# brianz98/A-Fortran-Electronic-Structure-Program

Hardware: AMD Instinct MI355X
Metric: CCSD iter wall-time (s) + (T) wall-time (s); fp64 TFLOP/s vs MFMA peak (higher is better)
Workload: dtype f64; 1 GPU; cfg5: nocc=20 nvirt=200, synthetic hashed ERIs scale 0.005; step = 1 CCSD iteration (replicated) + full (T) over i<=j<=k sharded across ranks; nocc=20, nvirt=200, triples=1540, parallelism=(T) ijk-shard x1, CCSD replicas

## Files before the change

### a-fortran-electronic-structure-program_amd/csrc/ccsd.h

```cpp
#pragma once
#include "afesp_internal.h"

namespace afesp {

struct DiisRing {
    int nerr = 0, nact = 0, it = 0;
    int64_t nvec = 0;
    double *amp = nullptr;
    double *amp_s = nullptr;
    double *hist_t = nullptr, *hist_e = nullptr;
    double *coef = nullptr;
    double *bmat = nullptr;
    bool tail_pending = false;
    int tail_slot = 0, tail_n = 0;
    double tail_b[256];
};
void diis_alloc(Context& cx, DiisRing& r, int diis_nerr);
void diis_save(Context& cx, DiisRing& r);
void diis_update(Context& cx, DiisRing& r);

struct CCState : DiisRing {
    int o = 0, v = 0;
    bool ready = false;
    double* e = nullptr;
    Tensor v_oovv, v_ovov, v_vvov, v_oovo, v_oooo, v_vvvv, w_oovv, w_vvov, w_oovo;
    Tensor D1, D2, t1, t2, t2_old, r1, r2;
    double* pp = nullptr;
    double* r2_sh = nullptr;
    double* r1_sh = nullptr;
    bool sharded = false;
    int sh_rank = 0, sh_world = 1;
    int64_t* pp_tab = nullptr;
    bool pp_sym = false;
    double *pp_vs = nullptr, *pp_va = nullptr, *pp_cs = nullptr, *pp_ca = nullptr, *pp_ps = nullptr, *pp_pa = nullptr;
    int64_t pp_ks = 0, pp_ka = 0, pp_ns = 0, pp_na = 0, pp_kn = 0;
    int64_t pp_lds = 0, pp_lda = 0;
    double *pp_ts = nullptr, *pp_ta = nullptr;
    double *oo_vs = nullptr, *oo_va = nullptr;
    double *oo_xs = nullptr, *oo_xa = nullptr;
    bool cs_packed = false;
    double* r1x = nullptr;
    bool r1x_valid = false;
    int hist_plain = 0;
    bool amps_touched = true;
    int64_t pp_nm = 0;
    double *ov_ws = nullptr, *ov_wa = nullptr;
    Tensor I_vo, I_vv, I_oo_p, I_oo, c, asym, x_voov, I_oooo, I_ovov, I_voov, I_ooov_p;
    Tensor z_ooov;
    double energy = 0.0, energy_old = 0.0, rms = 0.0;
    void* tplan = nullptr;
    Tensor I_vovv_pp, I_ooov_pp;
    const double* eri_src = nullptr;
    double* eri_own = nullptr;
    bool have_cr = false;
    int64_t amp_epoch = 0, cr_epoch = 0;
    void* ring = nullptr;
    bool partials_live = false;
    int64_t frozen_id = 0;
};
void triples_plan_free(CCState& s);

bool ring_tg_applies(const CCState& s);
bool ring_tg_pack(Context& cx, CCState& s);
void ring_tg_intermediates(Context& cx, CCState& s);
void ring_tg_residual(Context& cx, CCState& s);
void ring_tg_materialize(Context& cx, CCState& s, const Tensor& I_ovov_out, const Tensor& I_voov_out);
bool ring_live(const CCState& s);
bool ring_res_live(const CCState& s);
void ring_res_clear(CCState& s);
void ring_invalidate(CCState& s);
void ring_reinit(CCState& s);
const double* ring_Y(const CCState& s);
void ring_free(Context& cx, CCState& s);

void ccsd_init(Context& cx, CCState& s, int o, int v, const double* eri_mo_dev, const double* e_host, int diis_nerr);
bool ccsd_can_reinit(const CCState& s, int o, int v, int diis_nerr);
void ccsd_need_vvvv(Context& cx, CCState& s);
void ccsd_refresh_sharding(Context& cx, CCState& s);
bool ccsd_uses_lanes(const CCState& s);
void ccsd_diis_save(Context& cx, CCState& s);
void ccsd_intermediates(Context& cx, CCState& s, bool save_for_diis = false);
void ccsd_amplitudes(Context& cx, CCState& s, bool defer_update = false);
void ccsd_tail_launch(Context& cx, CCState& s);
int ccsd_tail_read(Context& cx, CCState& s, double e_tol, double t_tol);
void ccsd_pp_ladder(Context& cx, CCState& s);
void ccsd_ooov_pair_form(Context& cx, CCState& s, double* out = nullptr, int64_t a0 = 0, int64_t a1 = 0);
const double* ccsd_residual_full(Context& cx, CCState& s, bool r2);
void ccsd_build_I_vovv_p(Context& cx, CCState& s, const Tensor& out);
// ... 16 lines not shown
```

### a-fortran-electronic-structure-program_amd/csrc/ccsd.hip

```cpp
#include <algorithm>
#include <cmath>
#include <cstdlib>
#include <cstring>

#include "ccsd.h"
#include "comm.h"
#include "fused.h"

namespace afesp {

static inline int64_t tri64(int64_t i, int64_t j) { return i >= j ? i * (i + 1) / 2 + j : j * (j + 1) / 2 + i; }

bool ccsd_can_reinit(const CCState& s, int o, int v, int diis_nerr)
{
    if (!knobs().cc_reinit) return false;
    return s.ready && s.o == o && s.v == v && s.nerr == diis_nerr && s.pp_sym == pp_sym_pays(o, v);
}

void ccsd_init(Context& cx, CCState& s, int o, int v, const double* eri_mo_dev, const double* e_host, int diis_nerr)
{
    if (o <= 0 || v <= 0) throw Error(1, "ccsd_init: need at least one occupied and one virtual orbital");
    const bool again = ccsd_can_reinit(s, o, v, diis_nerr);
    if (again) {
        cx.quiesce();
// ... 32 lines not shown
    const int64_t fid = ++cx.amp_clock;
    for (Tensor* t : {&s.v_oovv, &s.v_ovov, &s.v_vvov, &s.v_oovo, &s.v_oooo, &s.w_oovv, &s.w_oovo}) t->frozen = fid;
    s.frozen_id = fid;
    if (again && s.w_vvov.d) {
        k_antisym_pair(cx, s.w_vvov.d, s.v_vvov.d, s.v, s.v, s.o, s.v, 0);
        s.w_vvov.frozen = fid;
    }
    T(s.D1, {O, V}); T(s.D2, {O, O, V, V});
    k_denominators(cx, s.D1.d, s.D2.d, s.e, o, v);
    s.nvec = ov + o2v2;
    if (!again) {
        s.amp = cx.alloc(s.nvec);
        s.t1 = view(s.amp, {O, V}); s.t2 = view(s.amp + ov, {O, O, V, V});
        double* res = cx.alloc(s.nvec);
        s.r1 = view(res, {O, V}); s.r2 = view(res + ov, {O, O, V, V});
    } else {
        AFESP_HIP(hipMemsetAsync(s.t1.d, 0, sizeof(double) * ov, cx.stream));
        AFESP_HIP(hipMemsetAsync(s.t2_old.d, 0, sizeof(double) * o2v2, cx.stream));
    }
    T(s.t2_old, {O, O, V, V});
    T(s.I_vo, {V, O}); T(s.I_vv, {V, V}); T(s.I_oo_p, {O, O}); T(s.I_oo, {O, O});
    T(s.c, {O, O, V, V}); T(s.asym, {O, O, V, V}); T(s.x_voov, {V, O, O, V});
    T(s.I_oooo, {O, O, O, O}); T(s.I_ovov, {O, V, O, V}); T(s.I_voov, {V, O, O, V});
    T(s.I_ooov_p, {O, O, O, V}); T(s.z_ooov, {O, O, O, V});
    {
        const int64_t np = V * (V + 1) / 2, K2 = V * V, N2 = O * O;
        A(s.pp, N2 * np + O * O * V * V + O * V);
        s.r2_sh = s.pp + N2 * np;
        s.r1_sh = s.r2_sh + O * O * V * V;
        std::vector<int64_t> tab;
        if (!s.pp_sym) {
            tab.reserve((size_t)(np + 2 * K2 + N2));
            for (int64_t b = 0; b < V; ++b)
                for (int64_t a = 0; a <= b; ++a) tab.push_back((a + V * b) * K2);
            for (int64_t k = 0; k < K2; ++k) tab.push_back(k);
            for (int64_t k = 0; k < K2; ++k) tab.push_back(N2 * k);
            for (int64_t x = 0; x < N2; ++x) tab.push_back(x);
            for (int64_t pz = 0; pz < np; ++pz) tab.push_back(N2 * pz);
        } else {
            auto even = [](int64_t x) { return (x + 1) & ~(int64_t)1; };
            const int64_t npa = V * (V - 1) / 2, ks = even(np), ka = even(npa), ns = even(O * (O + 1) / 2), na = even(O * (O - 1) / 2);
            s.pp_ks = ks; s.pp_ka = ka; s.pp_ns = ns; s.pp_na = na;
            const int64_t lds = ks + ns, lda = ka + na, kx = lds;
            s.pp_lds = lds; s.pp_lda = lda;
            const int64_t nm = std::max(np, O * V);
            s.pp_nm = nm;
            A(s.pp_vs, lds * np); A(s.pp_cs, ns * kx); A(s.pp_ps, ns * nm);
// ... 39 lines not shown
    if (s.v_vvvv.d) return;
    if (!s.eri_src)
        throw Error(1, "the <ef|ab> slice is formed on request from the packed MO integrals, and those have been replaced since "
                       "afesp_ccsd_init: initialise the solver again");
    const int64_t V = s.v;
    s.v_vvvv = cx.tensor({V, V, V, V});
    k_slice_phys(cx, s.v_vvvv.d, s.eri_src, s.v, s.v, s.v, s.v, s.o, s.o, s.o, s.o);
}

static void ccsd_need_w_vvov(Context& cx, CCState& s)
{
    if (s.w_vvov.d) return;
    s.w_vvov = cx.tensor({(int64_t)s.v, (int64_t)s.v, (int64_t)s.o, (int64_t)s.v});
    k_antisym_pair(cx, s.w_vvov.d, s.v_vvov.d, s.v, s.v, s.o, s.v, 0);
    s.w_vvov.frozen = s.frozen_id;
}

void ccsd_free(Context& cx, CCState& s)
{
    if (!s.o) return;
    if (s.eri_own) cx.release(s.eri_own);
    double* bufs[] = {s.e, s.v_oovv.d, s.v_ovov.d, s.v_vvov.d, s.v_oovo.d, s.v_oooo.d, s.v_vvvv.d, s.w_oovv.d, s.w_vvov.d,
                      s.w_oovo.d, s.D1.d, s.D2.d, s.amp, s.r1.d, s.t2_old.d, s.I_vo.d, s.I_vv.d, s.I_oo_p.d, s.I_oo.d, s.c.d,
                      s.asym.d, s.x_voov.d, s.I_oooo.d, s.I_ovov.d, s.I_voov.d, s.I_ooov_p.d, s.z_ooov.d, s.amp_s, s.hist_t,
                      s.hist_e, s.coef, s.I_vovv_pp.d, s.I_ooov_pp.d, s.pp, (double*)s.pp_tab, s.pp_vs, s.pp_va, s.pp_cs,
                      s.pp_ca, s.pp_ps, s.pp_pa, s.bmat, s.ov_ws, s.ov_wa, s.pp_ts, s.pp_ta, s.oo_vs, s.oo_va, s.oo_xs, s.oo_xa, s.r1x};
    for (double* b : bufs) cx.release(b);
    if (cx.plans.size() > 1024 || cx.plan_bytes > ((size_t)4 << 30)) cx.plan_clear();
    cx.drop_scratch();
    triples_plan_free(s);
    ring_free(cx, s);
    s = CCState();
}

void diis_alloc(Context& cx, DiisRing& s, int diis_nerr)
{
    s.nerr = diis_nerr; s.nact = 0; s.it = 0;
    if (diis_nerr >= 2) {
        if (diis_nerr > 15) throw Error(1, "ccsd_init: ccsd_diis_n_errmat > 15 is not supported");
        s.amp_s = cx.alloc(s.nvec);
        s.hist_t = cx.alloc(s.nvec * diis_nerr);
        s.hist_e = cx.alloc(s.nvec * diis_nerr);
        s.coef = cx.alloc(32);
        s.bmat = cx.alloc((int64_t)diis_nerr * diis_nerr);
    }
}

// ... 27 lines not shown
        if (knobs().cc_time_slice) { s.sharded = true; s.sh_rank = knobs().cc_time_rank; s.sh_world = knobs().cc_time_world; }
}

static void slice_bounds(const CCState& s, int64_t* v0, int64_t* v1)
{
    if (!s.sharded) { *v0 = 0; *v1 = s.v; return; }
    *v0 = (int64_t)s.v * s.sh_rank / s.sh_world;
    *v1 = (int64_t)s.v * (s.sh_rank + 1) / s.sh_world;
}

static Tensor slice_axis(Tensor t, int axis, int64_t lo, int64_t hi)
{
    t.d += lo * t.stride[axis];
    t.dim[axis] = hi - lo;
    return t;
}

void ccsd_intermediates(Context& cx, CCState& s, bool save_for_diis)
{
    auto C = [&](double al, const Tensor& A, const char* la, const Tensor& B, const char* lb, double be, const Tensor& Cc,
                 const char* lc) { contract(cx, al, A, la, B, lb, be, Cc, lc); };
    ccsd_refresh_sharding(cx, s);
    s.amps_touched = false;
    s.r1x_valid = false;
    int64_t v0, v1;
    slice_bounds(s, &v0, &v1);
    auto sl = [&](const Tensor& t, int axis) { return slice_axis(t, axis, v0, v1); };
    if (!(lanes_pay(s) || cx.rec) && ring_tg_applies(s) && ring_tg_pack(cx, s)) {}
    else k_asym_c(cx, s.asym.d, s.c.d, s.t1.d, s.t2.d, s.o, s.v);
    const bool par = lanes_pay(s) && !cx.rec;
    const bool fused = cx.rec != nullptr;
    const bool ring = !par && !fused && ring_tg_applies(s);
    if (!ring) ring_invalidate(s);
    auto lane = [&](int i) { if (par) cx.use_lane(i); };
    if (par) cx.fork(6);
    lane(0);
    C(1.0, s.w_oovv, "miea", s.t1, "me", 0.0, s.I_vo, "ai");
    lane(1);
    const bool ivv_diag = !par && !fused && s.o >= 2;
    if (!ivv_diag) {
        ccsd_need_w_vvov(cx, s);
        C(1.0, s.w_vvov, "ebma", s.t1, "me", 0.0, s.I_vv, "ba");
    }
    if (!s.sharded) C(-1.0, s.w_oovv, "mneb", s.c, "mnea", ivv_diag ? 0.0 : 1.0, s.I_vv, "ba");
    else if (v1 > v0) C(-1.0, s.w_oovv, "mneb", sl(s.c, 3), "mnea", ivv_diag ? 0.0 : 1.0, slice_axis(s.I_vv, 1, v0, v1), "ba");
    lane(0);
// ... 7 lines not shown
    }
    C(1.0, s.t1, "je", s.I_vo, "ei", 1.0, s.I_oo, "ji");
    lane(1);
    k_copy(cx, s.I_oooo.d, s.v_oooo.d, s.I_oooo.size());
    if (s.pp_sym && !par && !fused) ccsd_oooo_pair_form(cx, s);
    else C(1.0, s.c, "klef", s.v_oovv, "ijef", 1.0, s.I_oooo, "klij");
    C(1.0, s.t1, "ke", s.v_oovo, "ilej", 1.0, s.I_oooo, "klij");
    C(1.0, s.t1, "le", s.v_oovo, "jkei", 1.0, s.I_oooo, "klij");
    lane(2);
    const int64_t a_len = s.I_ovov.stride[3], a_off = v0 * a_len, a_cnt = (v1 - v0) * a_len;
    if (ivv_diag && s.sharded) {
        if (v1 > v0) C(1.0, s.t1, "je", sl(s.v_vvov, 3), "ebia", 0.0, sl(s.I_ovov, 3), "jbia");
    } else if (ivv_diag) {
        contract_pair(cx, {1.0, &s.t1, "je", &s.v_vvov, "ebia", 0.0, &s.I_ovov, "jbia"}, {1.0, &s.v_vvov, "beia", &s.t1, "je", 0.0, &s.x_voov, "bjia"});
    } else if (v1 > v0) {
        k_copy(cx, s.I_ovov.d + a_off, s.v_ovov.d + a_off, a_cnt);
        if (!ring) C(-0.5, s.v_oovv, "mibe", sl(s.c, 2), "mjae", 1.0, sl(s.I_ovov, 3), "jbia");
        C(-1.0, s.v_oovo, "mibj", sl(s.t1, 1), "ma", 1.0, sl(s.I_ovov, 3), "jbia");
        C(1.0, s.t1, "je", sl(s.v_vvov, 3), "ebia", 1.0, sl(s.I_ovov, 3), "jbia");
    }
    lane(3);
    if (s.sharded) { if (v1 > v0) C(1.0, sl(s.v_vvov, 3), "beia", s.t1, "je", 0.0, sl(s.x_voov, 3), "bjia"); }
    else if (!ivv_diag) C(1.0, s.v_vvov, "beia", s.t1, "je", 0.0, s.x_voov, "bjia");
    if (ivv_diag && v1 > v0) {
        k_ivv_diag(cx, s.I_vv.d, s.I_ovov.d, s.x_voov.d, s.o, s.v, (int)v0, (int)v1);
        k_axpby(cx, s.I_ovov.d + a_off, 1.0, s.v_ovov.d + a_off, 1.0, a_cnt);
        if (!ring) C(-0.5, s.v_oovv, "mibe", sl(s.c, 2), "mjae", 1.0, sl(s.I_ovov, 3), "jbia");
        C(-1.0, s.v_oovo, "mibj", sl(s.t1, 1), "ma", 1.0, sl(s.I_ovov, 3), "jbia");
    }
    const int x_voov_ready = par ? cx.mark() : 0;
    if (v1 > v0) {
        permute_add(cx, 1.0, sl(s.v_oovv, 2), "jiab", 0.0, sl(s.I_voov, 3), "bjia");
        if (fused) C(1.0, s.v_vvov, "beia", s.t1, "je", 1.0, s.I_voov, "bjia");
        else k_axpby(cx, s.I_voov.d + a_off, 1.0, s.x_voov.d + a_off, 1.0, a_cnt);
        if (!ring) {
            C(0.5, s.w_oovv, "imbe", sl(s.t2, 3), "mjea", 1.0, sl(s.I_voov, 3), "bjia");
            C(-0.5, s.v_oovv, "imbe", sl(s.c, 2), "mjae", 1.0, sl(s.I_voov, 3), "bjia");
        }
        C(-1.0, s.v_oovo, "imbj", sl(s.t1, 1), "ma", 1.0, sl(s.I_voov, 3), "bjia");
    }
    if (ring) ring_tg_intermediates(cx, s);
    lane(4);
    if (save_for_diis) diis_save(cx, s);
    if (fused) permute_add(cx, 1.0, s.v_oovo, "kjai", 0.0, s.z_ooov, "jkia");
    C(1.0, s.t1, "ie", s.v_oovv, "mjeb", fused ? 1.0 : 0.0, s.z_ooov, "ijmb");
    C(1.0, s.t1, "je", s.v_ovov, "mbie", 1.0, s.z_ooov, "ijmb");
    lane(5);
    permute_add(cx, 1.0, s.v_oovo, "kjai", 0.0, s.I_ooov_p, "jkia");
    if (s.sharded) {
        Tensor osh = view(cx.scratch("ooov_sh", s.I_ooov_p.size()), {(int64_t)s.o, (int64_t)s.o, (int64_t)s.o, (int64_t)s.v});
        if (v1 > v0) {
            if (s.pp_sym) {
                AFESP_HIP(hipMemsetAsync(osh.d + osh.stride[3] * v0, 0, sizeof(double) * osh.stride[3] * (v1 - v0), cx.stream));
                ccsd_ooov_pair_form(cx, s, osh.d, v0, v1);
            } else {
                C(1.0, s.t2, "jkef", sl(s.v_vvov, 3), "efia", 0.0, sl(osh, 3), "jkia");
            }
            if (par) cx.wait(x_voov_ready);
            C(1.0, s.t1, "je", sl(s.x_voov, 3), "ekia", 1.0, sl(osh, 3), "jkia");
        }
    } else if (s.pp_sym) {
        ccsd_ooov_pair_form(cx, s);
    } else {
        C(1.0, s.t2, "jkef", s.v_vvov, "efia", 1.0, s.I_ooov_p, "jkia");
// ... 179 lines not shown
    if (par) {
        r2b.d = cx.scratch(R2_LANE2, s.r2.size());
        r2c.d = cx.scratch(R2_LANE3, s.r2.size());
        r1b.d = cx.scratch(R1_LANE5, s.r1.size());
        cx.fork(6);
    }
    lane(0);
    if (!sh) C(1.0, s.t1, "ie", s.I_vv, "ea", 0.0, s.r1, "ia");
    C(-1.0, s.I_oo_p, "im", s.t1, "ma", sh ? 0.0 : 1.0, s.r1, "ia");
    C(1.0, s.asym, "miea", s.I_vo, "em", 1.0, s.r1, "ia");
    C(2.0, s.v_oovv, "miea", s.t1, "me", 1.0, s.r1, "ia");
    lane(5);
    if (par && cx.test_throw == 1) {
        cx.test_throw = 0;
        throw Error(99, "injected failure (afesp_test_inject)");
    }
    C(-1.0, s.v_ovov, "maie", s.t1, "me", par ? 0.0 : 1.0, r1b, "ia");
    C(-1.0, s.v_oovo, "mien", s.asym, "mnea", 1.0, r1b, "ia");
    if (!sh && s.r1x_valid && !par && !cx.rec) k_axpby(cx, r1b.d, 1.0, s.r1x, 1.0, r1b.size());
    else if (!sh) C(1.0, s.asym, "mief", s.v_vvov, "efma", 1.0, r1b, "ia");
    lane(1);
    const bool open_with_vvov = !par && !cx.rec && !sh;
    if (ring) ring_tg_residual(cx, s);
    if (open_with_vvov && !s.amps_touched) permute_add(cx, 1.0, s.x_voov, "bija", ring ? 1.0 : 0.0, s.r2, "ijab");
    else if (open_with_vvov) C(1.0, s.t1, "ie", s.v_vvov, "baje", ring ? 1.0 : 0.0, s.r2, "ijab");
    if (!sh) {
        C(1.0, s.t2, "ijae", s.I_vv, "eb", open_with_vvov ? 1.0 : 0.0, s.r2, "ijab");
        C(-1.0, s.t2, "miba", s.I_oo, "jm", 1.0, s.r2, "ijab");
    }
    lane(4);
    ccsd_pp_ladder(cx, s);
    lane(1);
    if (!sh && !(s.pp_sym && !cx.rec)) C(0.5, s.I_oooo, "ijmn", s.c, "mnab", 1.0, s.r2, "ijab");
    lane(2);
    if (ring) {
    } else if (!sh) {
        C(-1.0, s.t2, "mjae", s.I_ovov, "iemb", par ? 0.0 : 1.0, r2b, "ijab");
        C(-1.0, s.I_ovov, "iema", s.t2, "mjeb", 1.0, r2b, "ijab");
    } else if (v1 > v0) {
        C(-1.0, s.t2, "mjae", sl(s.I_ovov, 3), "iemb", 1.0, sl(r2s, 3), "ijab");
        C(-1.0, sl(s.I_ovov, 3), "iema", s.t2, "mjeb", 1.0, sl(r2s, 2), "ijab");
        C(1.0, s.asym, "miea", sl(s.I_voov, 3), "ejmb", 1.0, sl(r2s, 3), "ijab");
        Tensor osh = view(cx.scratch("ooov_sh", s.I_ooov_p.size()), {(int64_t)s.o, (int64_t)s.o, (int64_t)s.o, (int64_t)s.v});
        C(-1.0, s.t1, "ma", sl(osh, 3), "ijmb", 1.0, sl(r2s, 3), "ijab");
        C(1.0, s.t1, "ie", slice_axis(s.v_vvov, 0, v0, v1), "baje", 1.0, sl(r2s, 3), "ijab");
        C(1.0, s.t2, "ijae", slice_axis(s.I_vv, 1, v0, v1), "eb", 1.0, sl(r2s, 3), "ijab");
        C(-1.0, slice_axis(s.t2, 2, v0, v1), "miba", s.I_oo, "jm", 1.0, sl(r2s, 3), "ijab");
        C(0.5, s.I_oooo, "ijmn", sl(s.c, 3), "mnab", 1.0, sl(r2s, 3), "ijab");
        C(-1.0, s.t1, "ma", sl(s.z_ooov, 3), "ijmb", 1.0, sl(r2s, 3), "ijab");
        Tensor r1s = s.r1;
        r1s.d = s.r1_sh;
        C(1.0, s.t1, "ie", slice_axis(s.I_vv, 1, v0, v1), "ea", 1.0, slice_axis(r1s, 1, v0, v1), "ia");
        C(1.0, s.asym, "mief", sl(s.v_vvov, 3), "efma", 1.0, slice_axis(r1s, 1, v0, v1), "ia");
    }
    lane(3);
    if (!sh && !ring) C(1.0, s.asym, "miea", s.I_voov, "ejmb", par ? 0.0 : 1.0, r2c, "ijab");
    if (!open_with_vvov && !sh) C(1.0, s.t1, "ie", s.v_vvov, "baje", 1.0, r2c, "ijab");
    if (!sh) C(-1.0, s.t1, "ma", s.z_ooov, "ijmb", 1.0, r2c, "ijab");
    if (par) cx.join();
    if (sh) {
        const int64_t np = (int64_t)s.v * (s.v + 1) / 2;
        comm_allreduce_dev(cx, cx.comm, s.pp, (int64_t)s.o * s.o * np + s.r2.size() + s.r1.size());
        k_copy(cx, s.r2.d, s.r2_sh, s.r2.size());
        k_axpby(cx, s.r1.d, 1.0, s.r1_sh, 1.0, s.r1.size());
    }
    if (defer_update) return;
    k_t2_update(cx, s.t2.d, s.r2.d, par ? r2b.d : nullptr, par ? r2c.d : nullptr, s.v_oovv.d, s.D2.d, s.pp, s.o, s.v, s.t1.d, s.r1.d,
                par ? r1b.d : nullptr, s.D1.d, ring ? ring_Y(s) : nullptr);
}

const double* ccsd_residual_full(Context& cx, CCState& s, bool r2)
{
    const int64_t n = r2 ? s.r2.size() : s.r1.size();
    double* full = cx.scratch(r2 ? "r2_full" : "r1_full", n);
    auto add_partial = [&](const char* buf) {
        auto it = cx.cache.find(buf);
        if (s.partials_live && it != cx.cache.end()) k_axpby(cx, full, 1.0, (const double*)it->second.first, 1.0, n);
    };
    if (r2) {
        k_r2_full(cx, full, s.r2.d, s.pp, s.o, s.v);
        add_partial(R2_LANE2);
// ... 215 lines not shown
```

### a-fortran-electronic-structure-program_amd/csrc/ring.hip

```cpp
#include <algorithm>
#include <cstdlib>
#include <cstring>

#include "ccsd.h"

namespace afesp {

struct RingTg {
    int64_t ov = 0, Kc = 0, each = 0;
    double* slab = nullptr;
    double *cp, *t2p, *t2x, *asp, *nIo, *Ivo, *F1, *F2, *F3, *Y;
    uint32_t* rc32 = nullptr;
    int64_t *cm1 = nullptr, *cn1 = nullptr, *cm2 = nullptr, *cn2 = nullptr;
    int64_t* tab_block = nullptr;
    TgGroup* groups = nullptr;
    int tiles = 0, mx = 0;
    bool pairs2 = false;
    bool frozen_built = false;
    bool packed = false;
    bool live = false;
    bool res_live = false;
};

__global__ __launch_bounds__(256) void ring_tables_kernel(uint32_t* rc32, int64_t* cm1, int64_t* cn1, int64_t* cm2, int64_t* cn2, int o, int v,
                                                          int64_t Kc)
{
    const int64_t ov = (int64_t)o * v;
    for (int64_t x = (int64_t)blockIdx.x * blockDim.x + threadIdx.x; x < ov + 256; x += (int64_t)gridDim.x * blockDim.x) {
        const int64_t y = x < ov ? x : ov - 1;
        rc32[x] = (uint32_t)(8 * Kc * y);
        if (x < ov + 128) {
            const int64_t p = y % o, q = y / o;
            cm1[x] = Kc * y;
            cn1[x] = y;
// ... 51 lines not shown
        int r2 = (int)ring_div((unsigned)r, inv_np);
        const int pp = r - r2 * np;
        const int qq = (int)ring_div((unsigned)r2, a.inv_o), j = r2 - qq * o;
        const int blk = oo * (pp + P * qq);
        const double t = tile[m + o * j + blk], tt = tile[j + o * m + blk];
        const int64_t out = m + O * (p0 + pp) + a.Kc * (j + O * (q0 + qq));
        a.t2p[out] = t;
        a.asp[out] = 2.0 * t - tt;
    }
    const unsigned inv_nq = nq == 1 ? 0u : (unsigned)(((uint64_t)1 << 32) / (unsigned)nq + 1);
    for (int idx = threadIdx.x; idx < n; idx += 256) {
        int r = (int)ring_div((unsigned)idx, a.inv_o);
        const int m = idx - r * o;
        int r2 = (int)ring_div((unsigned)r, inv_nq);
        const int qq = r - r2 * nq;
        const int pp = (int)ring_div((unsigned)r2, a.inv_o), j = r2 - pp * o;
        const double t = tile[m + o * j + oo * (pp + P * qq)];
        const int64_t out = m + O * (q0 + qq) + a.Kc * (j + O * (p0 + pp));
        a.t2x[out] = t;
        a.cp[out] = t + a.t1[m + o * (p0 + pp)] * a.t1[j + o * (q0 + qq)];
    }
}

static RingTg* ring_get(Context& cx, CCState& s)
{
    if (s.ring) return (RingTg*)s.ring;
    RingTg* r = new RingTg();
    s.ring = r;
    const int64_t O = s.o, V = s.v;
    r->ov = O * V;
    r->Kc = (r->ov + TG_BK - 1) / TG_BK * TG_BK;
    r->each = r->Kc * r->ov + 2 * TG_BK;
    r->each = (r->each + 15) / 16 * 16;
    r->slab = cx.alloc(10 * r->each);
    double** bufs[10] = {&r->cp, &r->t2p, &r->t2x, &r->asp, &r->nIo, &r->Ivo, &r->F1, &r->F2, &r->F3, &r->Y};
    for (int q = 0; q < 10; ++q) *bufs[q] = r->slab + q * r->each;
    const int64_t n32 = r->ov + 256, n64 = r->ov + 128;
    int64_t* tab = cx.alloc_i64(4 * n64 + (n32 + 1) / 2 + 8);
    r->cm1 = tab; r->cn1 = tab + n64; r->cm2 = tab + 2 * n64; r->cn2 = tab + 3 * n64;
    r->rc32 = (uint32_t*)(tab + 4 * n64);
    r->tab_block = tab;
    AFESP_KLAUNCH(ring_tables_kernel, dim3((unsigned)std::min<int64_t>((n32 + 255) / 256, 4096)), dim3(256), 0, cx.stream, r->rc32, r->cm1,
                       r->cn1, r->cm2, r->cn2, s.o, s.v, r->Kc);
    AFESP_HIP(hipGetLastError());
    const int M = (int)r->ov, mt = (M + TG_BM - 1) / TG_BM, nt = (M + TG_BN - 1) / TG_BN;
    const int nk1 = (int)(r->Kc / TG_BK), gm = tgemm_group_m(M, nt);
    r->mx = nt;
    r->tiles = 2 * mt * nt;
    auto off = [&](const double* p) { return (int64_t)(p - r->slab); };
    TgGroup g[6] = {};
    auto fill = [&](TgGroup& d, const double* a1, const double* a2, const double* b1, const double* b2, const double* c, const int64_t* cn,
                    int tile0, int nk) {
        d.a1 = off(a1); d.a2 = off(a2); d.b1 = off(b1); d.b2 = off(b2); d.c0 = off(c);
        d.colB = r->rc32; d.offCn = cn;
        d.N = M; d.ntiles = nt; d.tile_start = tile0; d.nk1 = nk1; d.nk = nk;
        d.inv_width = tgemm_inverse(gm * nt);
    };
    fill(g[0], r->t2p, r->cp, r->F2, r->F3, r->Ivo, r->cn1, 0, 2 * nk1);
    fill(g[1], r->cp, r->cp, r->F1, r->F1, r->nIo, r->cn1, mt * nt, nk1);
    g[2].tile_start = 2 * mt * nt;
    fill(g[3], r->t2p, r->Ivo, r->nIo, r->asp, s.r2.d, r->cn2, 0, 2 * nk1);
    fill(g[4], r->nIo, r->nIo, r->t2x, r->t2x, r->Y, r->cn2, mt * nt, nk1);
    g[5].tile_start = 2 * mt * nt;
    r->groups = (TgGroup*)cx.alloc((int64_t)(6 * sizeof(TgGroup) / (sizeof(double)) + 1));
    AFESP_HIP(hipMemcpyAsync(r->groups, g, sizeof(g), hipMemcpyHostToDevice, cx.stream));
    AFESP_HIP(hipStreamSynchronize(cx.stream));
    r->pairs2 = (O % 2 == 0);
    return r;
}

void ring_free(Context& cx, CCState& s)
{
    RingTg* r = (RingTg*)s.ring;
    if (!r) return;
    cx.release(r->slab);
    cx.release(r->tab_block);
    cx.release(r->groups);
    delete r;
    s.ring = nullptr;
}

bool ring_live(const CCState& s) { return s.ring && ((RingTg*)s.ring)->live; }
bool ring_res_live(const CCState& s) { return s.ring && ((RingTg*)s.ring)->res_live; }
void ring_res_clear(CCState& s) { if (s.ring) ((RingTg*)s.ring)->res_live = false; }
const double* ring_Y(const CCState& s) { return ((RingTg*)s.ring)->Y; }

static Tensor kview(const RingTg* r, double* buf, const CCState& s, int pos_m, int pos_p, int pos_x, int pos_e)
{
    Tensor t;
    t.d = buf;
    t.rank = 4;
    const int64_t O = s.o, V = s.v;
    t.dim[pos_m] = O; t.stride[pos_m] = 1;
    t.dim[pos_e] = V; t.stride[pos_e] = O;
    t.dim[pos_p] = O; t.stride[pos_p] = r->Kc;
    t.dim[pos_x] = V; t.stride[pos_x] = r->Kc * O;
    return t;
}

bool ring_tg_pack(Context& cx, CCState& s)
{
    const bool off = !knobs().ring_pack;
    const int64_t oo = (int64_t)s.o * s.o;
    if (off || oo * 8 > 65536 || oo >= 65536 / 4) return false;
    RingTg* r = ring_get(cx, s);
    RingPackArgs a;
    a.t1 = s.t1.d; a.t2 = s.t2.d; a.asym = s.asym.d; a.c = s.c.d;
    a.cp = r->cp; a.t2p = r->t2p; a.t2x = r->t2x; a.asp = r->asp;
    a.o = s.o; a.v = s.v; a.Kc = r->Kc;
    a.P = a.Q = oo * 16 * 8 <= 65536 ? 4 : oo * 4 * 8 <= 65536 ? 2 : 1;
    a.inv_o = tgemm_inverse(s.o);
    a.inv_oo = tgemm_inverse((int)oo);
    const int tiles = ((s.v + a.P - 1) / a.P) * ((s.v + a.Q - 1) / a.Q);
    AFESP_KLAUNCH(ring_pack_kernel, dim3((unsigned)tiles), dim3(256), (size_t)(oo * a.P * a.Q * 8), cx.stream, a);
    AFESP_HIP(hipGetLastError());
    r->packed = true;
    return true;
}

void ring_tg_intermediates(Context& cx, CCState& s)
{
    RingTg* r = ring_get(cx, s);
    if (!r->frozen_built) {
        permute_add(cx, 0.5, s.v_oovv, "mibe", 0.0, kview(r, r->F1, s, 0, 1, 2, 3), "mibe");
        permute_add(cx, 0.5, s.w_oovv, "imbe", 0.0, kview(r, r->F2, s, 1, 0, 2, 3), "imbe");
        permute_add(cx, -0.5, s.v_oovv, "imbe", 0.0, kview(r, r->F3, s, 1, 0, 2, 3), "imbe");
        r->frozen_built = true;
    }
    if (!r->packed) {
        permute_add(cx, 1.0, s.c, "mjae", 0.0, kview(r, r->cp, s, 0, 1, 2, 3), "mjae");
        permute_add(cx, 1.0, s.t2, "mjea", 0.0, kview(r, r->t2p, s, 0, 1, 3, 2), "mjea");
        permute_add(cx, 1.0, s.t2, "mjae", 0.0, kview(r, r->t2x, s, 0, 1, 2, 3), "mjae");
        permute_add(cx, 1.0, s.asym, "miea", 0.0, kview(r, r->asp, s, 0, 1, 3, 2), "miea");
    }
    r->packed = false;
    const int ktail4 = (int)((r->ov - (r->Kc - TG_BK) + 3) / 4);
    TgProblem p{r->slab, r->slab, r->slab, r->rc32, r->cm1, (int)r->ov, true, ktail4};
    p.tag = 1;
    AFESP_HIP(tgemm_launch(p, r->groups, 2, r->tiles, r->mx, cx.stream, cx.tg));
    permute_add(cx, -1.0, s.I_ovov, "jbia", 1.0, kview(r, r->nIo, s, 2, 0, 3, 1), "jbia");
    permute_add(cx, 1.0, s.I_voov, "bjia", 1.0, kview(r, r->Ivo, s, 2, 1, 3, 0), "bjia");
    r->live = true;
}

void ring_tg_residual(Context& cx, CCState& s)
{
    RingTg* r = (RingTg*)s.ring;
    if (!r || !r->live) throw Error(2, "ring_tg_residual: the intermediates of this iteration were not formed on this path");
    const int ktail4 = (int)((r->ov - (r->Kc - TG_BK) + 3) / 4);
    TgProblem p{r->slab, r->slab, r->slab, r->rc32, r->cm2, (int)r->ov, r->pairs2, ktail4};
    p.tag = 1;
    AFESP_HIP(tgemm_launch(p, r->groups + 3, 2, r->tiles, r->mx, cx.stream, cx.tg));
    r->res_live = true;
}

void ring_tg_materialize(Context& cx, CCState& s, const Tensor& I_ovov_out, const Tensor& I_voov_out)
{
    RingTg* r = (RingTg*)s.ring;
    permute_add(cx, -1.0, kview(r, r->nIo, s, 2, 0, 3, 1), "jbia", 0.0, I_ovov_out, "jbia");
    permute_add(cx, 1.0, kview(r, r->Ivo, s, 2, 1, 3, 0), "bjia", 0.0, I_voov_out, "bjia");
}

void ring_reinit(CCState& s)
{
// ... 11 lines not shown
```

### a-fortran-electronic-structure-program_amd/csrc/solver.hip

```cpp
#include <cstdio>
#include <cstring>

#include "solver.h"
#include "integrals.h"

namespace afesp {

void GraphSlot::reset()
{
    if (exec) (void)hipGraphExecDestroy(exec);
    exec = nullptr;
    calls = 0;
    disabled = knobs().no_graph;
}

void Solver::cc_programs_reset(Context& cx)
{
    graph_cc.reset();
    fused_slot_reset(cx, fused_int);
    fused_slot_reset(cx, fused_amp);
    fused_slot_reset(cx, fused_iter);
}

void Solver::destroy(Context& cx)
// ... 183 lines not shown
    for (int it = 1; it <= maxiter; ++it) {
        const StepResult r = step(cx, e_tol, t_tol);
        record(it, r);
        if (r.converged) return it;
        ccsd_diis_update(cx, cc);
    }
    if (maxiter > 0) diis_check_flag(cx, host_scalars(cx, DIIS_FLAG_SLOT + 1));
    return -1;
}

void Solver::get_amplitudes(Context& cx, double* t1, double* t2)
{
    amps_to_host(cx, cc, t1, t2);
    diis_check_flag(cx, host_scalars(cx, DIIS_FLAG_SLOT + 1));
}

void Solver::set_amplitudes(Context& cx, const double* t1, const double* t2)
{
    cc.amp_epoch = ++cx.amp_clock;
    if (ring_live(cc)) {
        ring_tg_materialize(cx, cc, cc.I_ovov, cc.I_voov);
        ring_invalidate(cc);
    }
    cc.amps_touched = true;
    cc.tail_pending = false;
    if (t2) cc.hist_plain = cc.nerr + 1;
    amps_from_host(cx, cc, t1, t2);
}

void Solver::fetch_tensor(Context& cx, const char* name, double* out, int64_t capacity)
{
    CCState& s = cc;
    const int64_t O = s.o, V = s.v;
    struct { const char* n; const Tensor* t; } tab[] = {
        {"v_oovv", &s.v_oovv}, {"v_ovov", &s.v_ovov}, {"v_vvov", &s.v_vvov}, {"v_oovo", &s.v_oovo}, {"v_oooo", &s.v_oooo},
        {"v_vvvv", &s.v_vvvv}, {"I_vo", &s.I_vo}, {"I_vv", &s.I_vv}, {"I_oo_p", &s.I_oo_p}, {"I_oo", &s.I_oo},
        {"c_oovv", &s.c}, {"asym_t2", &s.asym}, {"x_voov", &s.x_voov}, {"I_oooo", &s.I_oooo}, {"I_ovov", &s.I_ovov},
        {"I_voov", &s.I_voov}, {"I_ooov_p", &s.I_ooov_p}, {"r1", &s.r1}, {"r2", &s.r2},
        {"D1", &s.D1}, {"D2", &s.D2}, {"t1", &s.t1}, {"t2", &s.t2}};
    auto is = [&](const char* n) { return !strcmp(name, n); };
    if (is("v_vvvv")) ccsd_need_vvvv(cx, s);
    Tensor vovv = view(nullptr, {V, O, V, V});
    const Tensor* t = is("I_vovv_p") ? &vovv : nullptr;
    for (auto& e : tab)
        if (is(e.n)) t = e.t;
    if (!t) throw Error(1, std::string("afesp_ccsd_get_tensor: unknown tensor ") + name);
// ... 157 lines not shown
```

Before: 60.12 TFLOP/s.

## Fuse small-o ring intermediate terms and residual I_oo/z terms into LDS-tiled kernels

Adds two LDS-tiled kernels for small occupied counts. The first folds the I_ovov/I_voov assembly (bare integral, t1 times v_oovo, permutation into the ring slab) into one pass per output. The second fuses the x_voov permute, the t2·I_oo contraction and the t1·z_ooov term of the r2 residual into one kernel. Precomputed G1/G2/W integral layouts are built once when the frozen integrals are set up. It also adds a t1 snapshot path that re-dresses z_ooov when amplitudes are set externally. This removes several separate permute and contraction launches and their memory round trips, at the cost of extra slab and W memory and more special-case code paths.

New measurement: 60.25 TFLOP/s (median of 6 runs). About the same (+0.2%).

```diff
diff --git a/a-fortran-electronic-structure-program_amd/csrc/ccsd.h b/a-fortran-electronic-structure-program_amd/csrc/ccsd.h
--- a/a-fortran-electronic-structure-program_amd/csrc/ccsd.h
+++ b/a-fortran-electronic-structure-program_amd/csrc/ccsd.h
@@ -43,6 +43,8 @@
     bool r1x_valid = false;
     int hist_plain = 0;
     bool amps_touched = true;
+    Tensor t1_im;
+    bool t1_im_valid = false;
     int64_t pp_nm = 0;
     double *ov_ws = nullptr, *ov_wa = nullptr;
     Tensor I_vo, I_vv, I_oo_p, I_oo, c, asym, x_voov, I_oooo, I_ovov, I_voov, I_ooov_p;
@@ -62,8 +64,11 @@
 
 bool ring_tg_applies(const CCState& s);
 bool ring_tg_pack(Context& cx, CCState& s);
-void ring_tg_intermediates(Context& cx, CCState& s);
+bool ring_tg_small_fused(const CCState& s);
+void ring_tg_intermediates(Context& cx, CCState& s, bool small_fused);
 void ring_tg_residual(Context& cx, CCState& s);
+bool ring_tg_residual_small_fits(const CCState& s);
+void ring_tg_residual_small(Context& cx, CCState& s);
 void ring_tg_materialize(Context& cx, CCState& s, const Tensor& I_ovov_out, const Tensor& I_voov_out);
 bool ring_live(const CCState& s);
 bool ring_res_live(const CCState& s);
diff --git a/a-fortran-electronic-structure-program_amd/csrc/ccsd.hip b/a-fortran-electronic-structure-program_amd/csrc/ccsd.hip
--- a/a-fortran-electronic-structure-program_amd/csrc/ccsd.hip
+++ b/a-fortran-electronic-structure-program_amd/csrc/ccsd.hip
@@ -78,7 +78,7 @@
     T(s.I_vo, {V, O}); T(s.I_vv, {V, V}); T(s.I_oo_p, {O, O}); T(s.I_oo, {O, O});
     T(s.c, {O, O, V, V}); T(s.asym, {O, O, V, V}); T(s.x_voov, {V, O, O, V});
     T(s.I_oooo, {O, O, O, O}); T(s.I_ovov, {O, V, O, V}); T(s.I_voov, {V, O, O, V});
-    T(s.I_ooov_p, {O, O, O, V}); T(s.z_ooov, {O, O, O, V});
+    T(s.I_ooov_p, {O, O, O, V}); T(s.z_ooov, {O, O, O, V}); T(s.t1_im, {O, V});
     {
         const int64_t np = V * (V + 1) / 2, K2 = V * V, N2 = O * O;
         A(s.pp, N2 * np + O * O * V * V + O * V);
@@ -164,7 +164,7 @@
     if (s.eri_own) cx.release(s.eri_own);
     double* bufs[] = {s.e, s.v_oovv.d, s.v_ovov.d, s.v_vvov.d, s.v_oovo.d, s.v_oooo.d, s.v_vvvv.d, s.w_oovv.d, s.w_vvov.d,
                       s.w_oovo.d, s.D1.d, s.D2.d, s.amp, s.r1.d, s.t2_old.d, s.I_vo.d, s.I_vv.d, s.I_oo_p.d, s.I_oo.d, s.c.d,
-                      s.asym.d, s.x_voov.d, s.I_oooo.d, s.I_ovov.d, s.I_voov.d, s.I_ooov_p.d, s.z_ooov.d, s.amp_s, s.hist_t,
+                      s.asym.d, s.x_voov.d, s.I_oooo.d, s.I_ovov.d, s.I_voov.d, s.I_ooov_p.d, s.z_ooov.d, s.t1_im.d, s.amp_s, s.hist_t,
                       s.hist_e, s.coef, s.I_vovv_pp.d, s.I_ooov_pp.d, s.pp, (double*)s.pp_tab, s.pp_vs, s.pp_va, s.pp_cs,
                       s.pp_ca, s.pp_ps, s.pp_pa, s.bmat, s.ov_ws, s.ov_wa, s.pp_ts, s.pp_ta, s.oo_vs, s.oo_va, s.oo_xs, s.oo_xa, s.r1x};
     for (double* b : bufs) cx.release(b);
@@ -238,6 +238,7 @@
                  const char* lc) { contract(cx, al, A, la, B, lb, be, Cc, lc); };
     ccsd_refresh_sharding(cx, s);
     s.amps_touched = false;
+    s.t1_im_valid = false;
     s.r1x_valid = false;
     int64_t v0, v1;
     slice_bounds(s, &v0, &v1);
@@ -291,14 +292,17 @@
     lane(3);
     if (s.sharded) { if (v1 > v0) C(1.0, sl(s.v_vvov, 3), "beia", s.t1, "je", 0.0, sl(s.x_voov, 3), "bjia"); }
     else if (!ivv_diag) C(1.0, s.v_vvov, "beia", s.t1, "je", 0.0, s.x_voov, "bjia");
-    if (ivv_diag && v1 > v0) {
+    const bool small_fused = ring && ivv_diag && ring_tg_small_fused(s);
+    if (ivv_diag && v1 > v0 && small_fused) {
+        k_ivv_diag(cx, s.I_vv.d, s.I_ovov.d, s.x_voov.d, s.o, s.v, (int)v0, (int)v1);
+    } else if (ivv_diag && v1 > v0) {
         k_ivv_diag(cx, s.I_vv.d, s.I_ovov.d, s.x_voov.d, s.o, s.v, (int)v0, (int)v1);
         k_axpby(cx, s.I_ovov.d + a_off, 1.0, s.v_ovov.d + a_off, 1.0, a_cnt);
         if (!ring) C(-0.5, s.v_oovv, "mibe", sl(s.c, 2), "mjae", 1.0, sl(s.I_ovov, 3), "jbia");
         C(-1.0, s.v_oovo, "mibj", sl(s.t1, 1), "ma", 1.0, sl(s.I_ovov, 3), "jbia");
     }
     const int x_voov_ready = par ? cx.mark() : 0;
-    if (v1 > v0) {
+    if (v1 > v0 && !small_fused) {
         permute_add(cx, 1.0, sl(s.v_oovv, 2), "jiab", 0.0, sl(s.I_voov, 3), "bjia");
         if (fused) C(1.0, s.v_vvov, "beia", s.t1, "je", 1.0, s.I_voov, "bjia");
         else k_axpby(cx, s.I_voov.d + a_off, 1.0, s.x_voov.d + a_off, 1.0, a_cnt);
@@ -308,7 +312,7 @@
         }
         C(-1.0, s.v_oovo, "imbj", sl(s.t1, 1), "ma", 1.0, sl(s.I_voov, 3), "bjia");
     }
-    if (ring) ring_tg_intermediates(cx, s);
+    if (ring) ring_tg_intermediates(cx, s, small_fused);
     lane(4);
     if (save_for_diis) diis_save(cx, s);
     if (fused) permute_add(cx, 1.0, s.v_oovo, "kjai", 0.0, s.z_ooov, "jkia");
@@ -534,11 +538,13 @@
     lane(1);
     const bool open_with_vvov = !par && !cx.rec && !sh;
     if (ring) ring_tg_residual(cx, s);
-    if (open_with_vvov && !s.amps_touched) permute_add(cx, 1.0, s.x_voov, "bija", ring ? 1.0 : 0.0, s.r2, "ijab");
+    const bool res_small = ring && open_with_vvov && !s.amps_touched && ring_tg_residual_small_fits(s);
+    if (res_small) ring_tg_residual_small(cx, s);
+    else if (open_with_vvov && !s.amps_touched) permute_add(cx, 1.0, s.x_voov, "bija", ring ? 1.0 : 0.0, s.r2, "ijab");
     else if (open_with_vvov) C(1.0, s.t1, "ie", s.v_vvov, "baje", ring ? 1.0 : 0.0, s.r2, "ijab");
     if (!sh) {
         C(1.0, s.t2, "ijae", s.I_vv, "eb", open_with_vvov ? 1.0 : 0.0, s.r2, "ijab");
-        C(-1.0, s.t2, "miba", s.I_oo, "jm", 1.0, s.r2, "ijab");
+        if (!res_small) C(-1.0, s.t2, "miba", s.I_oo, "jm", 1.0, s.r2, "ijab");
     }
     lane(4);
     ccsd_pp_ladder(cx, s);
@@ -568,7 +574,14 @@
     lane(3);
     if (!sh && !ring) C(1.0, s.asym, "miea", s.I_voov, "ejmb", par ? 0.0 : 1.0, r2c, "ijab");
     if (!open_with_vvov && !sh) C(1.0, s.t1, "ie", s.v_vvov, "baje", 1.0, r2c, "ijab");
-    if (!sh) C(-1.0, s.t1, "ma", s.z_ooov, "ijmb", 1.0, r2c, "ijab");
+    const bool redress = open_with_vvov && s.amps_touched && s.t1_im_valid;
+    if (redress) {
+        Tensor y = view(cx.scratch("z_redress", s.z_ooov.size()), {(int64_t)s.o, (int64_t)s.o, (int64_t)s.o, (int64_t)s.v});
+        C(1.0, s.t1, "ie", s.v_oovv, "mjeb", 0.0, y, "ijmb");
+        C(1.0, s.t1, "je", s.v_ovov, "mbie", 1.0, y, "ijmb");
+        C(-1.0, s.t1_im, "ma", y, "ijmb", 1.0, r2c, "ijab");
+        C(-1.0, s.t1, "ma", s.I_ooov_p, "ijmb", 1.0, r2c, "ijab");
+    } else if (!sh && !res_small) C(-1.0, s.t1, "ma", s.z_ooov, "ijmb", 1.0, r2c, "ijab");
     if (par) cx.join();
     if (sh) {
         const int64_t np = (int64_t)s.v * (s.v + 1) / 2;
diff --git a/a-fortran-electronic-structure-program_amd/csrc/ring.hip b/a-fortran-electronic-structure-program_amd/csrc/ring.hip
--- a/a-fortran-electronic-structure-program_amd/csrc/ring.hip
+++ b/a-fortran-electronic-structure-program_amd/csrc/ring.hip
@@ -10,6 +10,8 @@
     int64_t ov = 0, Kc = 0, each = 0;
     double* slab = nullptr;
     double *cp, *t2p, *t2x, *asp, *nIo, *Ivo, *F1, *F2, *F3, *Y;
+    double *G1 = nullptr, *G2 = nullptr;
+    double* W = nullptr;
     uint32_t* rc32 = nullptr;
     int64_t *cm1 = nullptr, *cn1 = nullptr, *cm2 = nullptr, *cn2 = nullptr;
     int64_t* tab_block = nullptr;
@@ -107,6 +109,270 @@
     }
 }
 
+struct RingSmallArgs {
+    const double *src, *fix, *w, *t1;
+    double* out;
+    int o, v, B, J, SB, SJ, nat, nbt;
+    int64_t Kc;
+    double sign;
+};
+constexpr int ring_small_a(int mode) { return mode == 0 ? 4 : 8; }
+constexpr int RING_SMALL_LDS = 4096, RING_SMALL_LDS_MAX = 7680;
+constexpr int RING_KU = 4;
+static int ring_ku_pad(int o) { return (o + RING_KU - 1) / RING_KU * RING_KU; }
+
+template <int MODE>
+__global__ __launch_bounds__(256) void ring_small_kernel(RingSmallArgs a)
+{
+    extern __shared__ double tile[];
+    constexpr int A = ring_small_a(MODE);
+    const int o = a.o, v = a.v;
+    const int at = (int)blockIdx.x % a.nat, rest = (int)blockIdx.x / a.nat, bt = rest % a.nbt, jt = rest / a.nbt;
+    const int a0 = at * A, b0 = bt * a.B, j0 = jt * a.J;
+    const int na = min(A, v - a0), nb = min(a.B, v - b0), nj = min(a.J, o - j0);
+    const int SA = a.SJ * a.J;
+    const int64_t O = o, V = v;
+    constexpr int KU = RING_KU, U = 4;
+    const double* __restrict__ src = a.src;
+    const double* __restrict__ fix = a.fix;
+    double* __restrict__ out = a.out;
+    double* t1s = tile + SA * A;
+    const int op = (o + KU - 1) / KU * KU;
+    for (int idx = threadIdx.x; idx < op * A; idx += 256) {
+        const int m = idx / A, aa = idx % A;
+        t1s[idx] = aa < na && m < o ? a.t1[m + O * (a0 + aa)] : 0.0;
+    }
+    const unsigned inv_o = o == 1 ? 0u : (unsigned)(((uint64_t)1 << 32) / (unsigned)o + 1);
+    const unsigned inv_nb = nb == 1 ? 0u : (unsigned)(((uint64_t)1 << 32) / (unsigned)nb + 1);
+    const unsigned inv_nj = nj == 1 ? 0u : (unsigned)(((uint64_t)1 << 32) / (unsigned)nj + 1);
+    const int n = o * nb * nj * na;
+    for (int base = threadIdx.x; base < n; base += 256 * U) {
+        double val[U];
+        int dst[U];
+#pragma unroll
+        for (int u = 0; u < U; ++u) {
+            const int idx = base + 256 * u;
+            dst[u] = -1;
+            val[u] = 0.0;
+            if (idx < n) {
+                int bb, jj, r;
+                if (MODE == 0) {
+                    r = (int)ring_div((unsigned)idx, inv_nj); jj = idx - r * nj;
+                    const int r2 = (int)ring_div((unsigned)r, inv_nb); bb = r - r2 * nb; r = r2;
+                } else {
+                    r = (int)ring_div((unsigned)idx, inv_nb); bb = idx - r * nb;
+                    const int r2 = (int)ring_div((unsigned)r, inv_nj); jj = r - r2 * nj; r = r2;
+                }
+                const int aa = (int)ring_div((unsigned)r, inv_o), i = r - aa * o;
+                const int64_t from = MODE == 0 ? (j0 + jj) + O * ((b0 + bb) + V * (i + O * (a0 + aa))) : (b0 + bb) + V * ((j0 + jj) + O * (i + O * (a0 + aa)));
+                dst[u] = i + a.SB * bb + a.SJ * jj + SA * aa;
+                val[u] = src[from];
+            }
+        }
+#pragma unroll
+        for (int u = 0; u < U; ++u)
+            if (dst[u] >= 0) tile[dst[u]] = val[u];
+    }
+    __syncthreads();
+    const int nx = o * nb * nj;
+    const int64_t N = O * V * O;
+    for (int x = threadIdx.x; x < nx; x += 256) {
+        const int r = (int)ring_div((unsigned)x, inv_o), i = x - r * o;
+        const int jj = (int)ring_div((unsigned)r, inv_nb), bb = r - jj * nb;
+        const double* __restrict__ w = a.w + (i + O * ((b0 + bb) + V * (j0 + jj)));
+        const int64_t to = (i + O * (b0 + bb)) + a.Kc * ((j0 + jj) + O * a0);
+        double fv[A], ov[A];
+#pragma unroll
+        for (int aa = 0; aa < A; ++aa) {
+            const int64_t q = to + a.Kc * O * aa;
+            fv[aa] = aa < na ? fix[q] : 0.0;
+            ov[aa] = aa < na ? out[q] : 0.0;
+        }
+        double acc[A] = {};
+        for (int m0 = 0; m0 < o; m0 += KU) {
+            double wv[KU];
+#pragma unroll
+            for (int u = 0; u < KU; ++u) wv[u] = m0 + u < o ? w[N * (m0 + u)] : 0.0;
+#pragma unroll
+            for (int u = 0; u < KU; ++u)
+#pragma unroll
+                for (int aa = 0; aa < A; ++aa) acc[aa] += wv[u] * t1s[A * (m0 + u) + aa];
+        }
+        const double* st = tile + (i + a.SB * bb + a.SJ * jj);
+#pragma unroll
+        for (int aa = 0; aa < A; ++aa)
+            if (aa < na) out[to + a.Kc * O * aa] = ov[aa] + a.sign * (st[SA * aa] + fv[aa] - acc[aa]);
+    }
+}
+
+static bool ring_small_plan(int o, int mode, int* B, int* J, int* SB, int* SJ)
+{
+    const int A = ring_small_a(mode);
+    *SB = o | 1;
+    if (mode == 0) {
+        *J = o;
+        *B = 8;
+        while (*B > 1 && ((*SB * *B) | 1) * o * A > RING_SMALL_LDS) --*B;
+    } else {
+        *B = 16;
+        *J = std::max(1, std::min(o, RING_SMALL_LDS / (((*SB * *B) | 1) * A)));
+    }
+    *SJ = (*SB * *B) | 1;
+    return *SJ * *J * A + ring_ku_pad(o) * A <= RING_SMALL_LDS_MAX;
+}
+
+bool ring_tg_small_fused(const CCState& s)
+{
+    int B, J, SB, SJ;
+    return s.o >= 2 && ring_small_plan(s.o, 0, &B, &J, &SB, &SJ) && ring_small_plan(s.o, 1, &B, &J, &SB, &SJ);
+}
+
+static void ring_small_launch(Context& cx, CCState& s, const RingTg* r, int mode)
+{
+    RingSmallArgs a;
+    ring_small_plan(s.o, mode, &a.B, &a.J, &a.SB, &a.SJ);
+    a.src = mode == 0 ? s.I_ovov.d : s.x_voov.d;
+    a.fix = mode == 0 ? r->G1 : r->G2;
+    a.w = r->W + (mode == 0 ? 0 : (int64_t)s.o * s.o * s.o * s.v);
+    a.t1 = s.t1.d;
+    a.out = mode == 0 ? r->nIo : r->Ivo;
+    a.sign = mode == 0 ? -1.0 : 1.0;
+    a.o = s.o; a.v = s.v; a.Kc = r->Kc;
+    const int A = ring_small_a(mode);
+    a.nat = (s.v + A - 1) / A;
+    a.nbt = (s.v + a.B - 1) / a.B;
+    const int64_t blocks = (int64_t)a.nat * a.nbt * ((s.o + a.J - 1) / a.J);
+    const size_t lds = sizeof(double) * ((size_t)a.SJ * a.J * A + (size_t)ring_ku_pad(s.o) * A);
+    if (mode == 0) AFESP_KLAUNCH(ring_small_kernel<0>, dim3((unsigned)blocks), dim3(256), lds, cx.stream, a);
+    else AFESP_KLAUNCH(ring_small_kernel<1>, dim3((unsigned)blocks), dim3(256), lds, cx.stream, a);
+    AFESP_HIP(hipGetLastError());
+}
+
+struct RingResArgs {
+    const double *x, *t2, *ioo, *t1, *z;
+    double* r2;
+    int o, v, B, SBB, nat, njt, ntile;
+};
+constexpr int RING_RES_A = 4, RING_RES_J = 4, RING_RES_B = 8, RING_XCDS = 8;
+
+__global__ __launch_bounds__(256) void ring_res_small_kernel(RingResArgs a)
+{
+    extern __shared__ double tile[];
+    constexpr int A = RING_RES_A, J = RING_RES_J;
+    const int o = a.o, v = a.v;
+    const int k = (int)blockIdx.x / RING_XCDS, jt = k % a.njt, t = (k / a.njt) * RING_XCDS + (int)blockIdx.x % RING_XCDS;
+    if (t >= a.ntile) return;
+    const int at = t % a.nat, bt = t / a.nat;
+    const int a0 = at * A, b0 = bt * a.B, j0 = jt * J;
+    const int na = min(A, v - a0), nb = min(a.B, v - b0), nj = min(J, o - j0);
+    const int nc = o * nj, ST = o * J;
+    const int64_t O = o, V = v;
+    constexpr int KU = RING_KU, U = 4;
+    const double* __restrict__ xs = a.x;
+    double* __restrict__ r2 = a.r2;
+    const int op = (o + KU - 1) / KU * KU;
+    double* t1s = tile + a.SBB * a.B;
+    double* ios = t1s + op * A;
+    for (int idx = threadIdx.x; idx < op * A; idx += 256) {
+        const int m = idx / A, aa = idx % A;
+        t1s[idx] = aa < na && m < o ? a.t1[m + O * (a0 + aa)] : 0.0;
+    }
+    for (int idx = threadIdx.x; idx < op * J; idx += 256) {
+        const int m = idx / J, jj = idx % J;
+        ios[idx] = jj < nj && m < o ? a.ioo[(j0 + jj) + O * m] : 0.0;
+    }
+    const unsigned inv_o = o == 1 ? 0u : (unsigned)(((uint64_t)1 << 32) / (unsigned)o + 1);
+    const unsigned inv_nb = nb == 1 ? 0u : (unsigned)(((uint64_t)1 << 32) / (unsigned)nb + 1);
+    const unsigned inv_nc = nc == 1 ? 0u : (unsigned)(((uint64_t)1 << 32) / (unsigned)nc + 1);
+    const unsigned inv_na = na == 1 ? 0u : (unsigned)(((uint64_t)1 << 32) / (unsigned)na + 1);
+    const int n = nb * nc * na;
+    for (int base = threadIdx.x; base < n; base += 256 * U) {
+        double val[U];
+        int dst[U];
+#pragma unroll
+        for (int u = 0; u < U; ++u) {
+            const int idx = base + 256 * u;
+            dst[u] = -1;
+            val[u] = 0.0;
+            if (idx < n) {
+                const int r = (int)ring_div((unsigned)idx, inv_nb), bb = idx - r * nb;
+                const int aa = (int)ring_div((unsigned)r, inv_nc), c = r - aa * nc;
+                dst[u] = c + ST * aa + a.SBB * bb;
+                val[u] = xs[(b0 + bb) + V * ((c + O * j0) + O * O * (a0 + aa))];
+            }
+        }
+#pragma unroll
+        for (int u = 0; u < U; ++u)
+            if (dst[u] >= 0) tile[dst[u]] = val[u];
+    }
+    __syncthreads();
+    const int n2 = o * na * nb;
+    for (int x = threadIdx.x; x < n2; x += 256) {
+        const int r = (int)ring_div((unsigned)x, inv_o), i = x - r * o;
+        const int bb = (int)ring_div((unsigned)r, inv_na), aa = r - bb * na;
+        const double* __restrict__ tp = a.t2 + (i + O * O * ((a0 + aa) + V * (b0 + bb)));
+        double acc[J] = {};
+        for (int m0 = 0; m0 < o; m0 += KU) {
+            double tv[KU];
+#pragma unroll
+            for (int u = 0; u < KU; ++u) tv[u] = m0 + u < o ? tp[O * (m0 + u)] : 0.0;
+#pragma unroll
+            for (int u = 0; u < KU; ++u)
+#pragma unroll
+                for (int jj = 0; jj < J; ++jj) acc[jj] += tv[u] * ios[J * (m0 + u) + jj];
+        }
+        double* st = tile + (i + ST * aa + a.SBB * bb);
+#pragma unroll
+        for (int jj = 0; jj < J; ++jj)
+            if (jj < nj) st[o * jj] -= acc[jj];
+    }
+    __syncthreads();
+    const int n3 = nc * nb;
+    for (int x = threadIdx.x; x < n3; x += 256) {
+        const int bb = (int)ring_div((unsigned)x, inv_nc), c = x - bb * nc;
+        const double* __restrict__ zp = a.z + ((c + O * j0) + O * O * O * (b0 + bb));
+        double* __restrict__ out = r2 + ((c + O * j0) + O * O * (a0 + V * (b0 + bb)));
+        double ov[A];
+#pragma unroll
+        for (int aa = 0; aa < A; ++aa) ov[aa] = aa < na ? out[O * O * aa] : 0.0;
+        double acc[A] = {};
+        for (int m0 = 0; m0 < o; m0 += KU) {
+            double zv[KU];
+#pragma unroll
+            for (int u = 0; u < KU; ++u) zv[u] = m0 + u < o ? zp[O * O * (m0 + u)] : 0.0;
+#pragma unroll
+            for (int u = 0; u < KU; ++u)
+#pragma unroll
+                for (int aa = 0; aa < A; ++aa) acc[aa] += zv[u] * t1s[A * (m0 + u) + aa];
+        }
+        const double* st = tile + (c + a.SBB * bb);
+#pragma unroll
+        for (int aa = 0; aa < A; ++aa)
+            if (aa < na) out[O * O * aa] = ov[aa] + (st[ST * aa] - acc[aa]);
+    }
+}
+
+static int ring_res_sbb(int o) { return (o * RING_RES_J * RING_RES_A) | 1; }
+
+bool ring_tg_residual_small_fits(const CCState& s)
+{
+    return ring_res_sbb(s.o) * RING_RES_B + ring_ku_pad(s.o) * (RING_RES_A + RING_RES_J) <= RING_SMALL_LDS_MAX;
+}
+
+void ring_tg_residual_small(Context& cx, CCState& s)
+{
+    RingResArgs a;
+    a.x = s.x_voov.d; a.t2 = s.t2.d; a.ioo = s.I_oo.d; a.t1 = s.t1.d; a.z = s.z_ooov.d; a.r2 = s.r2.d;
+    a.o = s.o; a.v = s.v; a.B = RING_RES_B; a.SBB = ring_res_sbb(s.o);
+    a.nat = (s.v + RING_RES_A - 1) / RING_RES_A;
+    a.njt = (s.o + RING_RES_J - 1) / RING_RES_J;
+    a.ntile = a.nat * ((s.v + a.B - 1) / a.B);
+    const int64_t blocks = (int64_t)((a.ntile + RING_XCDS - 1) / RING_XCDS) * RING_XCDS * a.njt;
+    const size_t lds = sizeof(double) * ((size_t)a.SBB * a.B + (size_t)ring_ku_pad(s.o) * (RING_RES_A + RING_RES_J));
+    AFESP_KLAUNCH(ring_res_small_kernel, dim3((unsigned)blocks), dim3(256), lds, cx.stream, a);
+    AFESP_HIP(hipGetLastError());
+}
+
 static RingTg* ring_get(Context& cx, CCState& s)
 {
     if (s.ring) return (RingTg*)s.ring;
@@ -117,9 +383,11 @@
     r->Kc = (r->ov + TG_BK - 1) / TG_BK * TG_BK;
     r->each = r->Kc * r->ov + 2 * TG_BK;
     r->each = (r->each + 15) / 16 * 16;
-    r->slab = cx.alloc(10 * r->each);
-    double** bufs[10] = {&r->cp, &r->t2p, &r->t2x, &r->asp, &r->nIo, &r->Ivo, &r->F1, &r->F2, &r->F3, &r->Y};
-    for (int q = 0; q < 10; ++q) *bufs[q] = r->slab + q * r->each;
+    const bool small = ring_tg_small_fused(s);
+    r->slab = cx.alloc((small ? 12 : 10) * r->each);
+    double** bufs[12] = {&r->cp, &r->t2p, &r->t2x, &r->asp, &r->nIo, &r->Ivo, &r->F1, &r->F2, &r->F3, &r->Y, &r->G1, &r->G2};
+    for (int q = 0; q < (small ? 12 : 10); ++q) *bufs[q] = r->slab + q * r->each;
+    if (small) r->W = cx.alloc(2 * O * O * O * V);
     const int64_t n32 = r->ov + 256, n64 = r->ov + 128;
     int64_t* tab = cx.alloc_i64(4 * n64 + (n32 + 1) / 2 + 8);
     r->cm1 = tab; r->cn1 = tab + n64; r->cm2 = tab + 2 * n64; r->cn2 = tab + 3 * n64;
@@ -159,6 +427,7 @@
     RingTg* r = (RingTg*)s.ring;
     if (!r) return;
     cx.release(r->slab);
+    if (r->W) cx.release(r->W);
     cx.release(r->tab_block);
     cx.release(r->groups);
     delete r;
@@ -203,10 +472,18 @@
     return true;
 }
 
-void ring_tg_intermediates(Context& cx, CCState& s)
+void ring_tg_intermediates(Context& cx, CCState& s, bool small_fused)
 {
     RingTg* r = ring_get(cx, s);
+    if (small_fused && !r->W) throw Error(2, "ring_tg_intermediates: the state was not set up for the one-pass small terms");
     if (!r->frozen_built) {
+        if (small_fused) {
+            const int64_t O = s.o, V = s.v;
+            permute_add(cx, 1.0, s.v_ovov, "jbia", 0.0, kview(r, r->G1, s, 2, 0, 3, 1), "jbia");
+            permute_add(cx, 1.0, s.v_oovv, "jiab", 0.0, kview(r, r->G2, s, 2, 1, 3, 0), "bjia");
+            permute_add(cx, 1.0, s.v_oovo, "mibj", 0.0, view(r->W, {O, V, O, O}), "ibjm");
+            permute_add(cx, 1.0, s.v_oovo, "imbj", 0.0, view(r->W + O * O * O * V, {O, V, O, O}), "ibjm");
+        }
         permute_add(cx, 0.5, s.v_oovv, "mibe", 0.0, kview(r, r->F1, s, 0, 1, 2, 3), "mibe");
         permute_add(cx, 0.5, s.w_oovv, "imbe", 0.0, kview(r, r->F2, s, 1, 0, 2, 3), "imbe");
         permute_add(cx, -0.5, s.v_oovv, "imbe", 0.0, kview(r, r->F3, s, 1, 0, 2, 3), "imbe");
@@ -223,8 +500,13 @@
     TgProblem p{r->slab, r->slab, r->slab, r->rc32, r->cm1, (int)r->ov, true, ktail4};
     p.tag = 1;
     AFESP_HIP(tgemm_launch(p, r->groups, 2, r->tiles, r->mx, cx.stream, cx.tg));
-    permute_add(cx, -1.0, s.I_ovov, "jbia", 1.0, kview(r, r->nIo, s, 2, 0, 3, 1), "jbia");
-    permute_add(cx, 1.0, s.I_voov, "bjia", 1.0, kview(r, r->Ivo, s, 2, 1, 3, 0), "bjia");
+    if (small_fused) {
+        ring_small_launch(cx, s, r, 0);
+        ring_small_launch(cx, s, r, 1);
+    } else {
+        permute_add(cx, -1.0, s.I_ovov, "jbia", 1.0, kview(r, r->nIo, s, 2, 0, 3, 1), "jbia");
+        permute_add(cx, 1.0, s.I_voov, "bjia", 1.0, kview(r, r->Ivo, s, 2, 1, 3, 0), "bjia");
+    }
     r->live = true;
 }
 
diff --git a/a-fortran-electronic-structure-program_amd/csrc/solver.hip b/a-fortran-electronic-structure-program_amd/csrc/solver.hip
--- a/a-fortran-electronic-structure-program_amd/csrc/solver.hip
+++ b/a-fortran-electronic-structure-program_amd/csrc/solver.hip
@@ -229,6 +229,7 @@
         ring_tg_materialize(cx, cc, cc.I_ovov, cc.I_voov);
         ring_invalidate(cc);
     }
+    if (!cc.amps_touched && cc.t1_im.d) { k_copy(cx, cc.t1_im.d, cc.t1.d, cc.t1.size()); cc.t1_im_valid = true; }
     cc.amps_touched = true;
     cc.tail_pending = false;
     if (t2) cc.hist_plain = cc.nerr + 1;
```
